# VinAIResearch/COMBAT

Hardware: AMD Instinct MI355X
Metric: images/sec per alternated generator+surrogate step, CIFAR-10 bs=128, 1/2/4/8 GPU (higher is better)
Workload: dtype bf16; 1 GPU; train_generator.py --dataset cifar10 --pc 0.5 --noise_rate 0.08: alternated PreActResNet18 surrogate + UNet generator step (Phase C + Phase G, both Nesterov-SGD updates), bs=128 per GPU, on-device augmentation on; per_gpu_batch=128, global_batch=128, parallelism=dp1 (RCCL all-reduce of netC grads in Phase C, netG grads in Phase G), losses_finite=True, deterministic=True

## Files before the change

combat_amd/_lib.py:

```python
from __future__ import annotations

import ctypes as C
import os

HERE = os.path.dirname(os.path.abspath(__file__))
LIB_PATH = os.environ.get("COMBAT_HIP_LIB") or os.path.join(HERE, "libcombat_hip.so")

c_i32, c_i64, c_f32, c_vp = C.c_int32, C.c_int64, C.c_float, C.c_void_p


class ConvArgs(C.Structure):

    _fields_ = [
        ("N", c_i32), ("H", c_i32), ("W", c_i32), ("C", c_i32),
        ("P", c_i32), ("Q", c_i32), ("K", c_i32),
        ("R", c_i32), ("S", c_i32), ("stride", c_i32), ("pad", c_i32),
        ("mode", c_i32),
        ("src", c_vp), ("wpack", c_vp), ("kpad", c_i32), ("rows_pad", c_i32), ("dst", c_vp),
        ("pro_scale", c_vp), ("pro_shift", c_vp), ("pro_group_stride", c_i32), ("pro_act", c_i32),
        ("pro_slope", c_f32),
        ("bias", c_vp), ("add_pre", c_vp), ("mask_x", c_vp), ("mask_scale", c_vp), ("mask_shift", c_vp),
        ("mask_activated", c_i32), ("mask_group_stride", c_i32), ("mask_slope", c_f32), ("mask_mul_scale", c_i32),
        ("add_post", c_vp), ("tanh_out", c_i32),
        ("stats_kind", c_i32), ("stats", c_vp), ("xh_mean", c_vp), ("xh_rstd", c_vp),
# ... 91 lines not shown
    "combat_head_fwd": (C.c_int, [c_vp, c_i32, c_i32, c_i32, c_vp, c_vp, c_i32, c_vp, c_f32, c_vp, c_vp, c_vp, c_vp,
                                  c_vp, c_vp, c_vp]),
    "combat_head_bwd": (C.c_int, [c_vp, c_i32, c_i32, c_i32, c_vp, c_i32, c_vp, c_vp, c_f32, c_vp, c_vp, c_vp, c_vp,
                                  c_vp]),
    "combat_head_fwd_bwd": (C.c_int, [c_vp, c_i32, c_i32, c_i32, c_vp, c_vp, c_i32, c_vp, c_f32, c_vp, c_vp, c_vp, c_vp,
                                      c_vp, c_vp, c_vp, c_vp, c_vp]),
    "combat_head_bwd_weights": (C.c_int, [c_vp, c_vp, c_i32, c_i32, c_i32, c_i32, c_vp, c_vp, c_vp]),
    "combat_prune_sweep": (C.c_int, [c_vp, c_i32, c_vp, c_vp, c_vp, c_i32, c_i32, c_i32, c_vp, c_vp, c_vp, c_vp, c_vp]),
    "combat_feature_colsum": (C.c_int, [c_vp, c_i32, c_i32, c_vp, c_vp]),
    "combat_strip_superimpose": (C.c_int, [c_vp, c_i32, c_vp, c_i32, c_vp, c_i32, c_i32, c_i32, c_vp, c_vp]),
    "combat_strip_entropy": (C.c_int, [c_vp, c_i32, c_i32, c_i32, c_vp, c_vp]),
    "combat_nc_blend": (C.c_int, [c_vp, c_i32, c_vp, c_i32, c_vp, c_i32, c_i32, c_i32, c_i32, c_vp, c_vp, c_f32, c_vp, c_vp,
                                  c_vp]),
    "combat_nc_update": (C.c_int, [c_vp, c_vp, c_i32, c_vp, c_i32, c_vp, c_i32, c_i32, c_i32, c_i32, c_vp, c_i32, c_i32,
                                   c_vp, c_vp, c_vp, c_vp, c_f32, c_vp, c_f32, c_f32, c_f32, c_f32, c_vp, c_vp, c_vp, c_i32,
                                   c_vp, c_vp]),
    "combat_gradcam_seed": (C.c_int, [c_vp, c_vp, c_i32, c_i32, c_i32, c_i32, c_vp, c_vp, c_vp, c_vp]),
    "combat_gradcam_map": (C.c_int, [c_vp, c_vp, c_i32, c_i32, c_i32, c_i32, c_vp, c_vp, c_vp, c_vp]),
    "combat_comm_unique_id": (C.c_int, [c_vp]),
    "combat_comm_init_rank": (C.c_int, [C.POINTER(c_vp), c_i32, c_vp, c_i32]),
    "combat_comm_destroy": (C.c_int, [c_vp]),
    "combat_allreduce": (C.c_int, [c_vp, c_i64, c_i32, c_vp, c_vp]),
    "combat_sgd_nesterov": (C.c_int, [c_vp, c_vp, c_i32, c_i64, c_f32, c_f32, c_f32, c_f32, c_i32, c_vp]),
    "combat_image_to_c8": (C.c_int, [c_vp, c_i32, c_i32, c_vp, c_vp]),
    "combat_nhwc_to_nchw_f32": (C.c_int, [c_vp, c_i32, c_i32, c_i32, c_i32, c_i32, c_vp, c_vp]),
    "combat_nchw_to_nhwc_bf16": (C.c_int, [c_vp, c_i32, c_i32, c_i32, c_i32, c_i32, c_vp, c_vp]),
    "combat_memset_zero": (C.c_int, [c_vp, c_i64, c_vp]),
    "combat_copy3": (C.c_int, [c_vp, c_vp, c_i64, c_vp, c_vp, c_i64, c_vp, c_vp, c_i64, c_vp]),
    "combat_relu_mask": (C.c_int, [c_vp, c_vp, c_i64, c_vp, c_vp]),
    "combat_colsum": (C.c_int, [c_vp, c_i64, c_i32, c_i32, c_vp, c_vp]),
    "combat_log_terms": (C.c_int, [c_vp, c_vp, c_vp, c_i32, c_i32, c_vp, c_vp, c_vp, c_vp]),
    "combat_log_terms_tv": (C.c_int, [c_vp, c_vp, c_vp, c_vp, c_i32, c_i32, c_vp, c_vp, c_vp, c_vp]),
    "combat_maxpool2": (C.c_int, [c_vp, c_i32, c_i32, c_i32, c_i32, c_vp, c_vp]),
    "combat_elu_affine": (C.c_int, [c_vp, c_i64, c_i32, c_vp, c_vp, c_vp, c_vp]),
    "combat_affine_act": (C.c_int, [c_vp, c_i64, c_i32, c_vp, c_vp, c_i64, c_f32, c_vp, c_vp]),
    "combat_dct_u8": (C.c_int, [c_vp, c_vp, c_i32, c_i32, c_vp, c_vp]),
    "combat_linear_nhwc": (C.c_int, [c_vp, c_i32, c_i32, c_i32, c_i32, c_vp, c_vp, c_i32, c_vp, c_vp]),
    "combat_grid_head_fwd": (C.c_int, [c_vp, c_vp, c_vp, c_i32, c_i32, c_vp, c_vp]),
    "combat_wanet_grid": (C.c_int, [c_vp, c_vp, c_i32, c_i32, c_f32, c_vp, c_vp, c_vp]),
    "combat_warp_fwd": (C.c_int, [c_vp, c_vp, c_vp, c_i32, c_i32, c_i32, c_vp, c_vp]),
    "combat_warp_bwd": (C.c_int, [c_vp, c_vp, c_vp, c_vp, c_i32, c_i32, c_i32, c_i32, c_vp, c_vp]),
    "combat_warp_bwd_input": (C.c_int, [c_vp, c_vp, c_i32, c_i32, c_i32, c_vp, c_vp]),
    "combat_wanet_field_bwd": (C.c_int, [c_vp, c_i32, c_vp, c_vp, c_i32, c_i32, c_f32, c_f32, c_vp, c_vp, c_vp, c_i32, c_vp,
                                         c_vp, c_vp, c_vp, c_vp]),
    "combat_plan_create": (c_vp, []),
    "combat_plan_destroy": (None, [c_vp]),
# ... 45 lines not shown
```

combat_amd/csrc/capi.cpp:

```cpp
#include "combat_hip.h"

#include <hip/hip_runtime.h>

#include <atomic>
#include <cstdlib>
#include <mutex>
#include <unordered_map>

#define COMBAT_ABI_VERSION 21

extern "C" const char *combat_version(void) { return "combat_hip gfx950 abi17"; }
extern "C" int combat_abi_version(void) { return COMBAT_ABI_VERSION; }

static std::atomic<int> g_deterministic{-1};
bool combat_deterministic() {
    int v = g_deterministic.load(std::memory_order_relaxed);
    if (v < 0) {
        const char *e = getenv("COMBAT_DETERMINISTIC");
        v = e && e[0] == '1';
        g_deterministic.store(v, std::memory_order_relaxed);
    }
    return v != 0;
}
extern "C" void combat_set_deterministic(int on) { g_deterministic.store(on ? 1 : 0, std::memory_order_relaxed); }
extern "C" int combat_get_deterministic(void) { return combat_deterministic() ? 1 : 0; }

float *combat_stream_scratch(void *stream, size_t bytes) {
    constexpr size_t kBytes = 2u << 20;
    if (bytes > kBytes) return nullptr;
    static std::mutex mu;
    static std::unordered_map<void *, float *> regions;
    std::lock_guard<std::mutex> lock(mu);
// ... 11 lines not shown
```

combat_amd/csrc/common.hpp:

```cpp
#pragma once
#include <hip/hip_runtime.h>
#include <hip/hip_ext.h>
#include <stdint.h>

#include "combat_hip.h"

typedef __attribute__((ext_vector_type(8))) __bf16 bf16x8_t;
typedef __attribute__((ext_vector_type(4))) float f32x4_t;
typedef __attribute__((ext_vector_type(4))) short s16x4_t;
typedef __attribute__((ext_vector_type(4))) unsigned int u32x4_t;

namespace combat_launch {
extern thread_local hipEvent_t t_stop;
extern thread_local bool t_stop_used;
}
#define COMBAT_LAUNCH(kernel, grid, block, smem, stream, ...)                                             \
    do {                                                                                                  \
        if (hipEvent_t stop_ = combat_launch::t_stop) {                                                   \
            hipExtLaunchKernelGGL(kernel, grid, block, smem, stream, nullptr, stop_, 0, __VA_ARGS__);     \
            combat_launch::t_stop_used = true;                                                            \
        } else {                                                                                          \
            hipLaunchKernelGGL(kernel, grid, block, smem, stream, __VA_ARGS__);                           \
        }                                                                                                 \
    } while (0)
// ... 43 lines not shown
    u[2] = pack_bf16x2(v[4], v[5]);
    u[3] = pack_bf16x2(v[6], v[7]);
    return u;
}

__device__ __forceinline__ uint4 pack8(const float (&v)[8]) {
    uint4 u;
    u.x = pack_bf16x2(v[0], v[1]);
    u.y = pack_bf16x2(v[2], v[3]);
    u.z = pack_bf16x2(v[4], v[5]);
    u.w = pack_bf16x2(v[6], v[7]);
    return u;
}

__device__ __forceinline__ void load8f(const float *p, float (&v)[8]) {
    const float4 a = *reinterpret_cast<const float4 *>(p);
    const float4 b = *reinterpret_cast<const float4 *>(p + 4);
    v[0] = a.x; v[1] = a.y; v[2] = a.z; v[3] = a.w;
    v[4] = b.x; v[5] = b.y; v[6] = b.z; v[7] = b.w;
}

__device__ __forceinline__ float round_bf16(float f) { return bf16_bits_to_f32(f32_to_bf16_bits(f)); }

__device__ __forceinline__ uint4 hilo_pixel(float r, float g, float b) {
    const float hr = round_bf16(r), hg = round_bf16(g), hb = round_bf16(b);
    uint4 u;
    u.x = pack_bf16x2(hr, hg);
    u.y = pack_bf16x2(hb, r - hr);
    u.z = pack_bf16x2(g - hg, b - hb);
    u.w = 0;
    return u;
}

static inline hipStream_t as_stream(void *s) { return reinterpret_cast<hipStream_t>(s); }

bool combat_deterministic();
float *combat_stream_scratch(void *stream, size_t bytes);

static inline int ilog2_exact(int v) {
    if (v <= 0 || (v & (v - 1))) return -1;
    int s = 0;
    while ((1 << s) < v) ++s;
    return s;
}
```

combat_amd/csrc/elementwise.hip:

```cpp
#include "common.hpp"
#include "plan.hpp"

namespace {

__global__ __launch_bounds__(256) void pack_weights_kernel(const float *__restrict__ w, int K, int taps, int creal,
                                                           int C, int dup, __bf16 *__restrict__ wf, int rows_f,
                                                           int kpad_f, __bf16 *__restrict__ wd, int rows_d,
                                                           int kpad_d, int Kc) {
    const long nf = (long)rows_f * kpad_f;
    const long nd = wd ? (long)rows_d * kpad_d : 0;
    for (long t = (long)blockIdx.x * blockDim.x + threadIdx.x; t < nf + nd; t += (long)gridDim.x * blockDim.x) {
        if (t < nf) {
            const int n = (int)(t / kpad_f), k = (int)(t - (long)n * kpad_f);
            const int tap = k / C, c = k - tap * C;
            float v = 0.f;
            if (n < K && tap < taps) {
                int cm = -1;
                if (c < creal) cm = c;
                else if (dup && c < 2 * creal) cm = c - creal;
                if (cm >= 0) v = w[((long)n * taps + tap) * creal + cm];
            }
            wf[t] = (__bf16)v;
        } else {
            const long u = t - nf;
// ... 305 lines not shown
            up_taps(oy, H, y0, y1, wy0, wy1);
            const float wy = (y0 == iy ? wy0 : 0.f) + (y1 == iy ? wy1 : 0.f);
            if (wy == 0.f) continue;
            for (int ox = 2 * ix - 1; ox <= 2 * ix + 2; ++ox) {
                if (ox < 0 || ox >= Wo) continue;
                int x0, x1;
                float wx0, wx1;
                up_taps(ox, W, x0, x1, wx0, wx1);
                const float wx = (x0 == ix ? wx0 : 0.f) + (x1 == ix ? wx1 : 0.f);
                if (wx == 0.f) continue;
                const long off = ((img * Ho + oy) * Wo + ox) * C + c;
                float g[8], o[8];
                unpack8(*reinterpret_cast<const uint4 *>(d_out + off), g);
                unpack8(*reinterpret_cast<const uint4 *>(out + off), o);
                const float wgt = wy * wx;
#pragma unroll
                for (int e = 0; e < 8; ++e) acc[e] = fmaf(wgt * (o[e] > 0.f ? 1.f : 0.2f), g[e], acc[e]);
            }
        }
        *reinterpret_cast<uint4 *>(du + ((img * H + iy) * W + ix) * C + c) = pack8(acc);
    }
}

__global__ __launch_bounds__(256) void sgd_kernel(void *const *__restrict__ ptrs, const int64_t *__restrict__ sizes,
                                                  float lr, float mu, float wd, float gscale, int first) {
    const int t = blockIdx.y;
    float *__restrict__ p = reinterpret_cast<float *>(ptrs[3 * t]);
    const float *__restrict__ g = reinterpret_cast<const float *>(ptrs[3 * t + 1]);
    float *__restrict__ b = reinterpret_cast<float *>(ptrs[3 * t + 2]);
    const long n = sizes[t];
    for (long i = (long)blockIdx.x * blockDim.x + threadIdx.x; i < n; i += (long)gridDim.x * blockDim.x) {
        const float pv = p[i];
        const float gv = fmaf(wd, pv, g[i] * gscale);
        const float bv = first ? gv : fmaf(mu, b[i], gv);
        b[i] = bv;
        p[i] = pv - lr * fmaf(mu, bv, gv);
    }
}

__global__ __launch_bounds__(256) void linear_nhwc_kernel(const __bf16 *__restrict__ x, int h, int w, int C,
                                                          const float *__restrict__ Wt, const float *__restrict__ b,
                                                          int classes, float *__restrict__ logits) {
    __shared__ float red[256];
    const int img = blockIdx.x;
    const int in = C * h * w;
    for (int j = 0; j < classes; ++j) {
        float s = 0.f;
        for (int i = threadIdx.x; i < in; i += 256) {
            const int c = i / (h * w), r = i - c * h * w;
            s = fmaf((float)x[((long)img * h * w + r) * C + c], Wt[(long)j * in + i], s);
        }
        red[threadIdx.x] = s;
        __syncthreads();
        for (int o = 128; o > 0; o >>= 1) {
            if ((int)threadIdx.x < o) red[threadIdx.x] += red[threadIdx.x + o];
            __syncthreads();
        }
        if (threadIdx.x == 0) logits[(long)img * classes + j] = red[0] + b[j];
        __syncthreads();
// ... 364 lines not shown
                                  void *du, void *stream) {
    COMBAT_PLAN_HOOK(combat_unet_up_bwd, d_out, out, N, H, W, C, du);
    if (!d_out || !out || !du || N <= 0 || H <= 0 || W <= 0 || C <= 0 || (C & 7)) return COMBAT_EINVAL;
    COMBAT_LAUNCH(unet_up_bwd_kernel, dim3(grid_for((long)N * H * W * (C / 8), 8192)), dim3(256), 0,
                       as_stream(stream), reinterpret_cast<const __bf16 *>(d_out), reinterpret_cast<const __bf16 *>(out),
                       N, H, W, C, reinterpret_cast<__bf16 *>(du));
    CB_LAUNCH_CHECK();
    return COMBAT_OK;
}

extern "C" int combat_sgd_nesterov(const void *ptrs, const int64_t *sizes, int32_t count, int64_t max_size, float lr,
                                   float momentum, float weight_decay, float grad_scale, int32_t first_step,
                                   void *stream) {
    COMBAT_PLAN_HOOK(combat_sgd_nesterov, ptrs, sizes, count, max_size, lr, momentum, weight_decay, grad_scale, first_step);
    if (!ptrs || !sizes || count <= 0 || max_size <= 0) return COMBAT_EINVAL;
    long bx = (max_size + 255) / 256;
    if (bx > 4096) bx = 4096;
    COMBAT_LAUNCH(sgd_kernel, dim3((unsigned)bx, (unsigned)count), dim3(256), 0, as_stream(stream),
                       reinterpret_cast<void *const *>(ptrs), sizes, lr, momentum, weight_decay, grad_scale, first_step);
    CB_LAUNCH_CHECK();
    return COMBAT_OK;
}

extern "C" int combat_linear_nhwc(const void *x, int32_t n, int32_t h, int32_t w, int32_t C, const float *Wt,
                                  const float *b, int32_t classes, float *logits, void *stream) {
    COMBAT_PLAN_HOOK(combat_linear_nhwc, x, n, h, w, C, Wt, b, classes, logits);
    if (!x || !Wt || !b || !logits || n <= 0 || h <= 0 || w <= 0 || C <= 0 || classes <= 0) return COMBAT_EINVAL;
    COMBAT_LAUNCH(linear_nhwc_kernel, dim3(n), dim3(256), 0, as_stream(stream),
                       reinterpret_cast<const __bf16 *>(x), h, w, C, Wt, b, classes, logits);
    CB_LAUNCH_CHECK();
    return COMBAT_OK;
}
```

combat_amd/csrc/norm.hip:

```cpp
#include "common.hpp"
#include "plan.hpp"

namespace {

constexpr int kStageRows = 64;

__device__ __forceinline__ void reduce_rows(const float *__restrict__ part, int C, int c, long row0, int nrows,
                                            int ry, double &s1, double &s2) {
    s1 = 0.0;
    s2 = 0.0;
    if (c >= C) return;
    for (int r = ry; r < nrows; r += 32) {
        float u[8], v[8];
#pragma unroll
        for (int q = 0; q < 8; ++q) {
            const int rr = r + 4 * q < nrows ? r + 4 * q : r;
            const float *p = part + ((row0 + rr) * 2) * (long)C + c;
            u[q] = p[0];
            v[q] = p[C];
        }
#pragma unroll
        for (int q = 0; q < 8; ++q) {
            if (r + 4 * q < nrows) {
                s1 += (double)u[q];
// ... 88 lines not shown
        const double gm = a.gamma ? (double)a.gamma[c] : 1.0;
        const double mean = a.mean[o], rstd = a.rstd[o];
        const double m1 = s1 / a.count, m2 = s2 / a.count;
        a.ca[o] = (float)(gm * rstd);
        a.cb[o] = (float)(-gm * rstd * rstd * m2);
        a.cc[o] = (float)(gm * rstd * (mean * rstd * m2 - m1));
        if (a.dgamma) a.dgamma[c] = (float)s2;
        if (a.dbeta) a.dbeta[c] = (float)s1;
    }
}

__global__ void bn_eval_fold_kernel(const float *gamma, const float *beta, const float *rm, const float *rv,
                                    float eps, int C, float *scale, float *shift) {
    const int c = blockIdx.x * blockDim.x + threadIdx.x;
    if (c >= C) return;
    const float s = gamma[c] / sqrtf(rv[c] + eps);
    scale[c] = s;
    shift[c] = beta[c] - rm[c] * s;
}

__global__ void bn_eval_fold_batch_kernel(const combat_bn_desc *__restrict__ descs, float eps) {
    const combat_bn_desc d = descs[blockIdx.y];
    for (int c = blockIdx.x * blockDim.x + threadIdx.x; c < d.C; c += gridDim.x * blockDim.x) {
        const float s = d.gamma[c] / sqrtf(d.running_var[c] + eps);
        d.scale[c] = s;
        d.shift[c] = d.beta[c] - d.running_mean[c] * s;
    }
}

__global__ __launch_bounds__(256) void group_stats_kernel(const __bf16 *__restrict__ x, const __bf16 *__restrict__ dz,
                                                          int groups, int rows_per_group, int C, int parts_per_image,
                                                          const float *__restrict__ xh_mean,
                                                          const float *__restrict__ xh_rstd,
                                                          float *__restrict__ part) {
    const int nch = C >> 3;
    const long t = (long)blockIdx.x * blockDim.x + threadIdx.x;
    if (t >= (long)groups * nch) return;
    const int g = (int)(t / nch), c = (int)(t % nch) * 8;
    float s1[8], s2[8], hs[8], hh[8];
#pragma unroll
    for (int e = 0; e < 8; ++e) s1[e] = s2[e] = 0.f;
    if (dz) {
        const long img = parts_per_image > 0 ? g / parts_per_image : 0;
        load8f(xh_rstd + img * C + c, hs);
        load8f(xh_mean + img * C + c, hh);
    }
    for (int r = 0; r < rows_per_group; ++r) {
        const long off = ((long)g * rows_per_group + r) * C + c;
        float xv[8];
// ... 867 lines not shown
```

combat_amd/engine.py:

```python
from __future__ import annotations

import ctypes
import os
from typing import Dict, List, Optional, Tuple

import torch

from . import ops
from ._lib import STATS_PER_WORKGROUP, TILE_D128x32, TILE_D128x64, TILE_S128x64, CombatHipError, ConvArgs, lib
from .nets import UNET_LAYERS
from .ops import Affine, PackedConv, bf16

BATCH_STATS_ROWS = 0 if os.environ.get("COMBAT_STATS_PER_WAVE") == "1" else STATS_PER_WORKGROUP

f32 = torch.float32


def _p(t):
    return None if t is None else t.data_ptr()


class Plan:

    serial = False
# ... 336 lines not shown
        self.sgd_sizes = torch.tensor([self.total], dtype=torch.int64, device=dev)

    def _slice(self, base: torch.Tensor, name: str) -> torch.Tensor:
        o, n, _ = self.offsets[name]
        return base[o:o + n]

    def grad_phys(self, name: str) -> torch.Tensor:
        o, n, shape = self.offsets[name]
        g = self.grad[o:o + n]
        if len(shape) == 4:
            k, c, r, s = shape
            return g.view(k, r * s, c)
        return g.view(shape)

    def logical(self, base: torch.Tensor, name: str) -> torch.Tensor:
        o, n, shape = self.offsets[name]
        g = base[o:o + n]
        if len(shape) == 4:
            k, c, r, s = shape
            return g.view(k, r, s, c).permute(0, 3, 1, 2)
        return g.view(shape)

    zero_ev = None

    def zero_grad_behind(self) -> None:
        if Plan.serial:
            return
        main = torch.cuda.current_stream()
        aux = _aux_stream(main)
        ev = torch.cuda.Event()
        ev.record(main)
        aux.wait_event(ev)
        ops.check(lib.combat_memset_zero(self.grad.data_ptr(), self.total * 4, aux.cuda_stream), "zero_grad")
        self.zero_ev = torch.cuda.Event()
        self.zero_ev.record(aux)

    def sgd_step(self, lr: float, momentum: float = 0.9, weight_decay: float = 5e-4, grad_scale: float = 1.0):
        ops.sgd_nesterov(self.sgd_ptrs, self.sgd_sizes, 1, self.total, lr, momentum, weight_decay, grad_scale, False)




def _zero_grad_call(fp, st):
    ev = fp.zero_ev
    if ev is not None:
        fp.zero_ev = None
        torch.cuda.current_stream().wait_event(ev)
        return 0
    return lib.combat_memset_zero(fp.grad.data_ptr(), fp.total * 4, st)


_SHORT_WORKGROUPS = False


class short_workgroups:

    def __enter__(self):
        global _SHORT_WORKGROUPS
        self.prev, _SHORT_WORKGROUPS = _SHORT_WORKGROUPS, True

    def __exit__(self, *exc):
        global _SHORT_WORKGROUPS
        _SHORT_WORKGROUPS = self.prev


def _tile_preference(a) -> None:
# ... 205 lines not shown
    @flush_at_marks.setter
    def flush_at_marks(self, value: bool) -> None:
        value = bool(value)
        if value != self._flush_at_marks:
            for slot in getattr(self, "slots", {}).values():
                for k in [k for k in slot.plans if k.startswith("bwd")]:
                    del slot.plans[k]
        self._flush_at_marks = value

    def __init__(self, module: torch.nn.Module):
        self.module = module
        self.device = next(module.parameters()).device
        if self.device.type != "cuda":
            raise CombatHipError("combat_amd engines run on the GPU only (module is on %s); there is no CPU path"
                                 % self.device)
        self.fp = FlatParams(module)
        self.convs: List[PackedConv] = []
        self.slots: Dict[Tuple, Slot] = {}
        self._scratch = torch.empty(ops.norm_scratch_bytes(1, 512) // 4, dtype=f32, device=self.device)
        self.weights_dirty = True

    def mark_weights_dirty(self) -> None:
        self.weights_dirty = True

    def slot(self, name: str, n: int, hw: int) -> Slot:
        key = (name, n, hw)
        s = self.slots.get(key)
        if s is None:
            s = Slot(self.device, n, hw)
            self.slots[key] = s
        return s

    def _pc(self, weight, stride, pad, cin_pad, dup=False, need_dgrad=True, row_scale=None) -> PackedConv:
        pc = PackedConv(weight, stride, pad, cin_pad, dup_hilo=dup, need_dgrad=need_dgrad, row_scale=row_scale)
        self.convs.append(pc)
        return pc

    def refresh(self) -> None:
        if not self.weights_dirty:
            return
        self._pack_all()
        self._refresh_extra()
        self.weights_dirty = False

    def _pack_all(self) -> None:
        ptrs = tuple(pc.weight.data_ptr() for pc in self.convs)
        if getattr(self, "_pack_ptrs", None) != ptrs:
            masters = [pc.master() for pc in self.convs]
            if any(m.data_ptr() != q for m, q in zip(masters, ptrs)):
                self._pack_ptrs = None
                for pc in self.convs:
                    pc.pack()
                return
            from ._lib import PackDesc
            tab = (PackDesc * len(self.convs))()
            for d, pc, m in zip(tab, self.convs, masters):
                pc.fill_desc(d, m)
            self._pack_tab = torch.frombuffer(bytearray(bytes(tab)), dtype=torch.uint8).to(self.device)
            self._pack_ptrs = ptrs
        ops.check(lib.combat_pack_weights_batch(self._pack_tab.data_ptr(), len(self.convs),
                                                torch.cuda.current_stream().cuda_stream), "combat_pack_weights_batch")

    def _refresh_extra(self) -> None:
        pass

    FUSED_DIRECT_PX = 1024
    FUSED_MAX_ROWS = 256

    def _norm_scratch(self, plan: Plan, groups: int, c: int, rows: int) -> torch.Tensor:
        if rows > self.FUSED_MAX_ROWS and ops.norm_scratch_bytes(groups, c) > self._scratch.numel() * 4:
            self._scratch = torch.empty(ops.norm_scratch_bytes(groups, c) // 4, dtype=f32, device=self.device)
        plan.hold(self._scratch)
        return self._scratch

    def _conv_norm(self, plan: Plan, slot: Slot, key: str, src, dst, pc: PackedConv, *, groups: int,
                   gamma=None, beta=None, running=None, act_dst=None, slope: float = 0.0, defer: bool = False,
                   **conv_kw) -> NormState:
        n, p, q, c = dst.shape
        pq, m = p * q, n * p * q
        a = ops.conv_args(src, dst, pc, 0, workspace=plan.workspace(src.device), **conv_kw)
        a.stats_kind = 1 | (BATCH_STATS_ROWS if groups == 1 else 0)
        _tile_preference(a)
        rows, rpi = ops.conv_stats_layout(a)
        fused = (groups == 1) or (rpi > 0)
# ... 138 lines not shown

class PreActEngine(NetEngine):

    def __init__(self, module):
        super().__init__(module)
        m = module
        self.classes = m.linear.out_features
        self.stem = self._pc(m.conv1.weight.data, 1, 1, 8, dup=True)
        self.blocks: List[_Blk] = []
        self.bns: List[_BN] = []
        for li in range(1, 5):
            for bi, blk in enumerate(getattr(m, "layer%d" % li)):
                e = _Blk()
                e.prefix = "layer%d.%d." % (li, bi)
                e.stride, e.cin, e.planes = blk.stride, blk.conv1.in_channels, blk.conv1.out_channels
                e.bn1, e.bn2 = _BN(self, blk.bn1, e.prefix + "bn1"), _BN(self, blk.bn2, e.prefix + "bn2")
                e.conv1 = self._pc(blk.conv1.weight.data, blk.stride, 1, e.cin)
                e.conv2 = self._pc(blk.conv2.weight.data, 1, 1, e.planes)
                e.sc = self._pc(blk.shortcut[0].weight.data, blk.stride, 0, e.cin) if hasattr(blk, "shortcut") else None
                self.blocks.append(e)
                self.bns += [e.bn1, e.bn2]
        self.lin_w, self.lin_b = m.linear.weight.data, m.linear.bias.data

    def _refresh_extra(self):
        self.fold_bn()

    def fold_bn(self):
        ptrs = tuple(t.data_ptr() for bn in self.bns for t in (bn.gamma, bn.beta, bn.rm, bn.rv))
        if getattr(self, "_bn_ptrs", None) != ptrs:
            from ._lib import BnDesc
            tab = (BnDesc * len(self.bns))()
            for d, bn in zip(tab, self.bns):
                d.gamma, d.beta, d.running_mean, d.running_var = (t.data_ptr() for t in (bn.gamma, bn.beta, bn.rm, bn.rv))
                d.scale, d.shift, d.C = bn.escale.data_ptr(), bn.eshift.data_ptr(), bn.C
            self._bn_tab = torch.frombuffer(bytearray(bytes(tab)), dtype=torch.uint8).to(self.device)
            self._bn_ptrs = ptrs
        ops.check(lib.combat_bn_eval_fold_batch(self._bn_tab.data_ptr(), len(self.bns), 1e-5,
                                                torch.cuda.current_stream().cuda_stream), "combat_bn_eval_fold_batch")

    def head_bufs(self, slot: Slot):
        n = slot.N
        return dict(
            logits=slot.buf("logits", (n, self.classes), f32), dlogits=slot.buf("dlogits", (n, self.classes), f32),
            pooled=slot.buf("pooled", (n, self.lin_w.shape[1]), f32), loss=slot.buf("loss", (1,), f32, zero=True),
            correct=slot.buf("correct", (2,), torch.int32, zero=True),
            targets=slot.buf("targets", (n,), torch.int64, zero=True),
            targets2=slot.buf("targets2", (n,), torch.int64, zero=True))

    def input(self, slot: Slot) -> torch.Tensor:
        return slot.buf("x", (slot.N, slot.hw, slot.hw, 8))

    FWD_SHARED = ("stem", "logits", "dlogits", "pooled", "targets", "targets2") + tuple(
        "b%d.%s" % (b, s) for b in range(8) for s in ("y1", "out", "sc", "a1", "act")) + ("stem.act",)

    def forward_plan(self, slot: Slot, train: bool, loss_weight: float = 1.0, with_targets2: bool = False,
                     split_head: bool = False, head_bwd: bool = False, two_loss: bool = False, keep_raw_blocks=()) -> Plan:
        keep_raw_blocks = tuple(sorted(set(int(b) for b in keep_raw_blocks)))
        if keep_raw_blocks:
            if type(self) is not PreActEngine or train or two_loss:
# ... 1010 lines not shown
```

combat_amd/ops.py:

```python
from __future__ import annotations

import ctypes
from dataclasses import dataclass
from typing import Optional

import torch

from . import _lib
from ._lib import ConvArgs, WgradArgs, check, lib

bf16 = torch.bfloat16


def _p(t: Optional[torch.Tensor]):
    return None if t is None else t.data_ptr()


def _stream():
    return torch.cuda.current_stream().cuda_stream


def _round_up(v: int, m: int) -> int:
    return (v + m - 1) // m * m

# ... 435 lines not shown
                                  d_feat.data_ptr(), _stream()),
          "combat_gradcam_seed", "n=%d N=%d classes=%d C=%d" % (n, N, classes, c))


def gradcam_map(act, grad, n, cam, raw=None, weights=None) -> None:
    if act.dim() != 4 or act.shape != grad.shape or act.dtype != bf16 or grad.dtype != bf16 or act.shape[1] != act.shape[2] \
            or act.shape[0] < n or not act.is_contiguous() or not grad.is_contiguous():
        raise ValueError("gradcam_map: act and grad must be contiguous bf16 [>= n = %d][f][f][C] of one shape, got %s %s / %s %s"
                         % (n, act.dtype, tuple(act.shape), grad.dtype, tuple(grad.shape)))
    f, c = act.shape[1], act.shape[3]
    for name, v, size in (("cam", cam, n * 32 * 32), ("raw", raw, n * f * f), ("weights", weights, n * c)):
        if v is not None and (v.dtype != torch.float32 or v.numel() < size or not v.is_contiguous()):
            raise ValueError("gradcam_map: %s must be contiguous fp32 with at least %d elements, got %s %s"
                             % (name, size, v.dtype, tuple(v.shape)))
    check(lib.combat_gradcam_map(act.data_ptr(), grad.data_ptr(), n, f, c, 32, cam.data_ptr(), _p(raw), _p(weights), _stream()),
          "combat_gradcam_map", "n=%d f=%d C=%d" % (n, f, c))


def sgd_nesterov(ptrs, sizes, count, max_size, lr, momentum, weight_decay, grad_scale, first_step) -> None:
    check(lib.combat_sgd_nesterov(ptrs.data_ptr(), sizes.data_ptr(), count, max_size, lr, momentum, weight_decay,
                                  grad_scale, int(first_step), _stream()), "combat_sgd_nesterov", "count=%d" % count)


def image_to_c8(x, out_c8) -> None:
    n, _, hw, _ = x.shape
    check(lib.combat_image_to_c8(x.data_ptr(), n, hw, out_c8.data_ptr(), _stream()), "combat_image_to_c8")


def nhwc_to_nchw_f32(x, c, out) -> None:
    n, h, w, cc = x.shape
    check(lib.combat_nhwc_to_nchw_f32(x.data_ptr(), n, h, w, cc, c, out.data_ptr(), _stream()),
          "combat_nhwc_to_nchw_f32")


def nchw_to_nhwc_bf16(x, out) -> None:
    n, c, h, w = x.shape
    check(lib.combat_nchw_to_nhwc_bf16(x.data_ptr(), n, c, h, w, out.shape[-1], out.data_ptr(), _stream()),
          "combat_nchw_to_nhwc_bf16")


def colsum(x, c_out, out) -> None:
    c = x.shape[-1]
    check(lib.combat_colsum(x.data_ptr(), x.numel() // c, c, c_out, out.data_ptr(), _stream()), "combat_colsum")


def maxpool2(x, out) -> None:
# ... 20 lines not shown
```

combat_amd/step.py:

```python
from __future__ import annotations

import contextlib
import copy
import math
from dataclasses import dataclass, field
from types import SimpleNamespace
from typing import Dict, List, Optional

import os

import numpy as np
import torch

from . import ops, trigger
from ._lib import lib
from .augment import PostTensorTransform
from .dist import GradReducer, bucket_ranges
from .engine import (FreqEngine, PlanSeq, PreActEngine, UnetEngine, _zero_grad_call, f32, low_priority_stream,
                     short_workgroups)

BUCKETS = (8, 16, 32, 64, 128, 256, 512, 1024)


def bucket(n: int) -> int:
# ... 348 lines not shown
            self._trigger_c(x_ptr, nb, k1c, st)
        ops.check(lib.combat_augment_fwd(s.cat_src.data_ptr(), s.tab_i[1].data_ptr(), aug_ptr[0], n, hw,
                                         eC.input(s.sC_train).data_ptr(), None, st), "augment 0")
        pl["C_train_f"].run(prof)
        side = self._side_stream()
        side.wait_event(ev_fork)
        xK, xC = eK.input(s.sK_eval), eC.input(s.sC_eval)
        bd_ptr = s.bd.data_ptr()
        with torch.cuda.stream(side):
            s2 = side.cuda_stream
            self._trigger_g(x_ptr, n, k1g, s2)
            ev_bd = torch.cuda.Event()
            ev_bd.record()
            ops.check(lib.combat_augment_fwd(x_ptr, None, aug_ptr[1], n, hw, xK.data_ptr(), None, s2), "augment 1")
            ops.check(lib.combat_augment_fwd(bd_ptr, None, aug_ptr[4], n, hw, xK[n:].data_ptr(), None, s2), "augment 4")
            pl["K_eval_f"].run(prof)
            pl["K_bd_b"].run(prof)
            ops.check(lib.combat_augment_bwd(s.sK_bd.bufs["g.img"].data_ptr(), 8, aug_ptr[4], n, hw,
                                             s.d_bd2.data_ptr(), 0, s2), "augment 4 bwd")
            ev_side = torch.cuda.Event()
            ev_side.record()

        self._backward_allreduce(pl["C_train_b"], eC, prof)
        eC.fp.sgd_step(float(lr_c if lr_c is not None else opt.lr_C), grad_scale=1.0 / self.world)
        if not self.keep_grads:
            eC.fp.zero_grad_behind()
        eC.mark_weights_dirty()
        eC.refresh()

        torch.cuda.current_stream().wait_event(ev_bd)
        self._c_eval_inputs(x_ptr, bd_ptr, xC, aug_ptr, n, st)
        pl["C_eval_f"].run(prof)
        ev_late = torch.cuda.Event()
        ev_late.record()
        pl["C_bd_b"].run(prof)
        self._c_eval_grads(aug_ptr, n, st)
        with torch.cuda.stream(side):
            side.wait_event(ev_late)
            s2 = side.cuda_stream
            if not s.merge_c:
                ops.check(lib.combat_augment_fwd(x_ptr, None, aug_ptr[2], n, hw, eC.input(s.sC_met).data_ptr(), None, s2),
                          "augment 2")
                pl["C_met_f"].run(prof)
            if eF is not None:
                ops.check(lib.combat_dct_u8(bd_ptr, self.D.data_ptr(), n, hw, eF.input(s.sF).data_ptr(), s2), "dct")
                pl["F_f"].run(prof)
            self._log_terms(n, s2, s.sF.bufs["logits"] if eF is not None else None)
            ev_met = torch.cuda.Event()
            ev_met.record()
        torch.cuda.current_stream().wait_event(ev_side)
        self._gen_backward(x_ptr, n, k1g, st, prof)
        eG.fp.sgd_step(float(lr_g if lr_g is not None else opt.lr_G), grad_scale=1.0 / self.world)
        if not self.keep_grads:
            eG.fp.zero_grad_behind()
        eG.mark_weights_dirty()
        torch.cuda.current_stream().wait_event(ev_met)
        self.samples += n
        self.steps_done += 1

    def _draw(self, targets_cpu, bd_targets_cpu) -> StepRandomness:
        return draw_randomness(targets_cpu, bd_targets_cpu, self.opt, self.transforms, self.sigma_range)

    def _gen_forward(self, x_ptr, n, st, prof) -> None:
        s = self.cur
        ops.check(lib.combat_image_to_c8(x_ptr, n, self.hw, self.eG.input(s.sG).data_ptr(), st), "c8 G")
        s.pl["G_f"].run(prof)

    def _trigger_c(self, x_ptr, nb, k1c, st) -> None:
        s = self.cur
        ops.check(lib.combat_trigger_fwd(x_ptr, self.eG.output(s.sG).data_ptr(), self.P.data_ptr(), k1c, float(self.opt.noise_rate),
                                         nb, self.hw, s.tab_i[0].data_ptr(), s.cat_src[s.n:].data_ptr(), None, None, st),
                  "trigger C")

    def _trigger_g(self, x_ptr, n, k1g, s2) -> None:
        s = self.cur
        ops.check(lib.combat_trigger_fwd(x_ptr, self.eG.output(s.sG).data_ptr(), self.P.data_ptr(), k1g, float(self.opt.noise_rate),
                                         n, self.hw, None, s.bd.data_ptr(), None, s.mse.data_ptr(), s2), "trigger G")

# ... 459 lines not shown
            g = self.eG.forward_grid(hw, float(opt.grid_rescale), st)
            ops.check(lib.combat_warp_fwd(s.cat_src.data_ptr(), s.tab_i[0].data_ptr(), g["grid"].data_ptr(), 0, nb, hw,
                                          s.cat_src[n:].data_ptr(), st), "warp")
        elif nb:
            self.eG.refresh()
            nbk = min(bucket(nb), n)
            if nbk not in self._small:
                small = self.eG.slot("V.small", nbk, hw)
                self._small[nbk] = (small, self.eG.forward_plan(small), torch.zeros(nbk, 3, hw, hw, dtype=f32, device=self.dev))
            sS, plan_small, tochange = self._small[nbk]
            self.k1.copy_(torch.from_numpy(trigger.gaussian_kernel1d(
                trigger.sample_sigma(getattr(opt, "sigma", (0.1, 1.0))), opt.kernel_size)))
            ops.check(lib.combat_augment_fwd(s.cat_src.data_ptr(), s.tab_i[0].data_ptr(), None, nbk, hw,
                                             self.eG.input(sS).data_ptr(), tochange.data_ptr(), st), "gather poisoned")
            plan_small.run()
            ops.check(lib.combat_trigger_fwd(tochange.data_ptr(), self.eG.output(sS).data_ptr(), self.P.data_ptr(),
                                             self.k1.data_ptr(), float(opt.noise_rate), nb, hw, None,
                                             s.cat_src[n:].data_ptr(), None, None, st), "trigger")
        ops.check(lib.combat_augment_fwd(s.cat_src.data_ptr(), s.tab_i[1].data_ptr(),
                                         s.tab_f.data_ptr() if aug is not None else None, n, hw,
                                         self.eC.input(s.slot).data_ptr(), None, st), "augment")
        s.fwd.run()
        backward_allreduce(s.bwd, self.eC, self.pg, self.world, self._reducers)
        self.eC.fp.sgd_step(float(lr if lr is not None else opt.lr_C), grad_scale=1.0 / self.world)
        self.eC.mark_weights_dirty()

    def poisoned_pair(self):
        trg, nb = getattr(self, "last_poisoned", (None, 0))
        if not nb:
            return None
        s = self.cur
        return s.cat_src[:s.n][trg.to(self.dev)].clone(), s.cat_src[s.n:s.n + nb].clone()

    def read_metrics(self, reset=False):
        out = {"loss_sum": 0.0, "correct": 0}
        for s in self._sets.values():
            h = self.eC.head_bufs(s.slot)
            out["loss_sum"] += float(h["loss"])
            out["correct"] += int(h["correct"][0])
            if reset:
                h["loss"].zero_()
                h["correct"].zero_()
        return out
```

include/combat_hip.h:

```cpp
#ifndef COMBAT_HIP_H
#define COMBAT_HIP_H

#include <stdint.h>

#ifdef __cplusplus
extern "C" {
#endif

#define COMBAT_OK 0
#define COMBAT_EINVAL (-1)
#define COMBAT_ELAUNCH (-2)

const char *combat_version(void);
int combat_abi_version(void);

void combat_set_deterministic(int on);
int combat_get_deterministic(void);

typedef struct combat_conv_args {
    int32_t N, H, W, C;
    int32_t P, Q, K;
    int32_t R, S, stride, pad;
    int32_t mode;
    const void *src;
// ... 214 lines not shown

int combat_strip_superimpose(const void *backgrounds, int32_t B, const void *dataset, int32_t n_data, const int32_t *index,
                             int32_t S, int32_t hw, int32_t norm_cols, void *out_c8, void *stream);
int combat_strip_entropy(const float *logits, int32_t B, int32_t S, int32_t classes, float *out, void *stream);

int combat_nc_blend(const void *dataset, int32_t n_data, const int32_t *index, int32_t n_index, const int32_t *cursor,
                    int32_t bs, int32_t n, int32_t N, int32_t hw, const float *mask_tanh, const float *pattern_tanh,
                    float epsilon, const float *norm, void *out_c8, void *stream);
int combat_nc_update(const void *g_img, const void *dataset, int32_t n_data, const int32_t *index, int32_t n_index,
                     int32_t *cursor, int32_t bs, int32_t n, int32_t N, int32_t hw, const float *logits, int32_t classes,
                     int32_t target_label, float *mask_tanh, float *pattern_tanh, float *exp_avg, float *exp_avg_sq,
                     float epsilon, const float *norm, float lr, float beta1, float beta2, float adam_eps, int32_t *t,
                     const float *cost, float *stats, int32_t steps, float *grad_out, void *stream);

int combat_gradcam_seed(const float *logits, const int32_t *index, int32_t n, int32_t N, int32_t classes, int32_t C,
                        const float *W, int32_t *chosen, void *d_feat, void *stream);
int combat_gradcam_map(const void *act, const void *grad, int32_t n, int32_t f, int32_t C, int32_t out_hw, float *cam,
                       float *raw, float *weights, void *stream);

int combat_sgd_nesterov(const void *ptrs, const int64_t *sizes, int32_t count, int64_t max_size, float lr,
                        float momentum, float weight_decay, float grad_scale, int32_t first_step,
                        void *stream);

int combat_image_to_c8(const float *x, int32_t n, int32_t hw, void *out_c8, void *stream);
int combat_nhwc_to_nchw_f32(const void *x, int32_t n, int32_t h, int32_t w, int32_t C, int32_t c, float *out,
                            void *stream);
int combat_nchw_to_nhwc_bf16(const float *x, int32_t n, int32_t c, int32_t h, int32_t w, int32_t C, void *out,
                             void *stream);
int combat_relu_mask(const void *g, const void *act, int64_t elements, void *out, void *stream);
int combat_memset_zero(void *ptr, int64_t bytes, void *stream);
int combat_copy3(void *dst0, const void *src0, int64_t bytes0, void *dst1, const void *src1, int64_t bytes1,
                 void *dst2, const void *src2, int64_t bytes2, void *stream);
int combat_colsum(const void *x, int64_t rows, int32_t C, int32_t c_out, float *out, void *stream);
int combat_log_terms(const float *x, const float *xb, const float *mse_partial, int32_t n, int32_t hw,
                     const float *detector_logits, double *acc2, double *hits, void *stream);
int combat_log_terms_tv(const float *x, const float *xb, const float *mse_partial, const float *tv_partial, int32_t n,
                        int32_t hw, const float *detector_logits, double *acc3, double *hits, void *stream);
int combat_maxpool2(const void *x, int32_t n, int32_t h, int32_t w, int32_t C, void *out, void *stream);
int combat_elu_affine(const void *x, int64_t rows, int32_t C, const float *scale, const float *shift, void *out,
                      void *stream);
int combat_affine_act(const void *x, int64_t rows, int32_t C, const float *scale, const float *shift,
                      int64_t group_rows, float slope, void *out, void *stream);
int combat_dct_u8(const float *x, const float *D, int32_t n, int32_t hw, void *out_c8, void *stream);
int combat_linear_nhwc(const void *x, int32_t n, int32_t h, int32_t w, int32_t C, const float *W, const float *b,
                       int32_t classes, float *logits, void *stream);

// ... 39 lines not shown
```

Before: 33150 images/sec.

## Fuse Nesterov SGD update with bf16 weight packing, BN fold and grad zeroing

Adds a single kernel that applies the Nesterov SGD update to the fp32 master weights and, in the same pass, writes the packed bf16 forward and transposed weight layouts, refolds the eval BatchNorm scale and shift, and zeros the gradients. Before, these were separate launches, each reading the full parameter set again. The later zero_grad call is skipped when the grad buffer was already cleared on the same stream. The price is a more complex kernel with a tiled transpose through shared memory and a fallback path for irregular convs, plus extra bookkeeping state (_fused_done, clean_on) that must stay consistent.

New measurement: 33240 images/sec, median of 5. Within noise of the previous version (+0.2%).

```diff
diff --git a/combat_amd/_lib.py b/combat_amd/_lib.py
--- a/combat_amd/_lib.py
+++ b/combat_amd/_lib.py
@@ -137,6 +137,8 @@
     "combat_comm_destroy": (C.c_int, [c_vp]),
     "combat_allreduce": (C.c_int, [c_vp, c_i64, c_i32, c_vp, c_vp]),
     "combat_sgd_nesterov": (C.c_int, [c_vp, c_vp, c_i32, c_i64, c_f32, c_f32, c_f32, c_f32, c_i32, c_vp]),
+    "combat_sgd_nesterov_pack": (C.c_int, [c_vp, c_vp, c_vp, c_i64, c_vp, c_i32, c_vp, c_i32, c_vp, c_i32, c_f32,
+                                           c_f32, c_f32, c_f32, c_f32, c_i32, c_i32, c_vp]),
     "combat_image_to_c8": (C.c_int, [c_vp, c_i32, c_i32, c_vp, c_vp]),
     "combat_nhwc_to_nchw_f32": (C.c_int, [c_vp, c_i32, c_i32, c_i32, c_i32, c_i32, c_vp, c_vp]),
     "combat_nchw_to_nhwc_bf16": (C.c_int, [c_vp, c_i32, c_i32, c_i32, c_i32, c_i32, c_vp, c_vp]),
diff --git a/combat_amd/csrc/capi.cpp b/combat_amd/csrc/capi.cpp
--- a/combat_amd/csrc/capi.cpp
+++ b/combat_amd/csrc/capi.cpp
@@ -7,7 +7,7 @@
 #include <mutex>
 #include <unordered_map>
 
-#define COMBAT_ABI_VERSION 21
+#define COMBAT_ABI_VERSION 22
 
 extern "C" const char *combat_version(void) { return "combat_hip gfx950 abi17"; }
 extern "C" int combat_abi_version(void) { return COMBAT_ABI_VERSION; }
diff --git a/combat_amd/csrc/common.hpp b/combat_amd/csrc/common.hpp
--- a/combat_amd/csrc/common.hpp
+++ b/combat_amd/csrc/common.hpp
@@ -89,6 +89,13 @@
 
 __device__ __forceinline__ float round_bf16(float f) { return bf16_bits_to_f32(f32_to_bf16_bits(f)); }
 
+__device__ __forceinline__ void bn_eval_fold_one(float gamma, float beta, float mean, float var, float eps, float &scale,
+                                                 float &shift) {
+    const float s = gamma / sqrtf(var + eps);
+    scale = s;
+    shift = beta - mean * s;
+}
+
 __device__ __forceinline__ uint4 hilo_pixel(float r, float g, float b) {
     const float hr = round_bf16(r), hg = round_bf16(g), hb = round_bf16(b);
     uint4 u;
diff --git a/combat_amd/csrc/elementwise.hip b/combat_amd/csrc/elementwise.hip
--- a/combat_amd/csrc/elementwise.hip
+++ b/combat_amd/csrc/elementwise.hip
@@ -351,6 +351,17 @@
     }
 }
 
+struct SgdScalars {
+    float lr, mu, wd, gscale;
+    int first;
+};
+
+__device__ __forceinline__ void sgd_update(const SgdScalars &s, float &p, float g, float &b) {
+    const float gv = fmaf(s.wd, p, g * s.gscale);
+    b = s.first ? gv : fmaf(s.mu, b, gv);
+    p = p - s.lr * fmaf(s.mu, b, gv);
+}
+
 __global__ __launch_bounds__(256) void sgd_kernel(void *const *__restrict__ ptrs, const int64_t *__restrict__ sizes,
                                                   float lr, float mu, float wd, float gscale, int first) {
     const int t = blockIdx.y;
@@ -358,12 +369,150 @@
     const float *__restrict__ g = reinterpret_cast<const float *>(ptrs[3 * t + 1]);
     float *__restrict__ b = reinterpret_cast<float *>(ptrs[3 * t + 2]);
     const long n = sizes[t];
+    const SgdScalars s{lr, mu, wd, gscale, first};
     for (long i = (long)blockIdx.x * blockDim.x + threadIdx.x; i < n; i += (long)gridDim.x * blockDim.x) {
-        const float pv = p[i];
-        const float gv = fmaf(wd, pv, g[i] * gscale);
-        const float bv = first ? gv : fmaf(mu, b[i], gv);
+        float pv = p[i], bv = b[i];
+        sgd_update(s, pv, g[i], bv);
         b[i] = bv;
-        p[i] = pv - lr * fmaf(mu, bv, gv);
+        p[i] = pv;
+    }
+}
+
+struct SgdPackArgs {
+    float *p, *g, *b;
+    const combat_pack_desc *descs;
+    const int64_t *segs;
+    const combat_bn_desc *bns;
+    int n_desc, n_seg, n_bn;
+    float eps;
+    int zero;
+    SgdScalars s;
+};
+
+__device__ __forceinline__ void sgd_one(const SgdPackArgs &a, long i) {
+    float pv = a.p[i], bv = a.b[i];
+    sgd_update(a.s, pv, a.g[i], bv);
+    a.b[i] = bv;
+    a.p[i] = pv;
+    if (a.zero) a.g[i] = 0.f;
+}
+
+__device__ __forceinline__ void store8f(float *p, const float (&v)[8]) {
+    *reinterpret_cast<float4 *>(p) = make_float4(v[0], v[1], v[2], v[3]);
+    *reinterpret_cast<float4 *>(p + 4) = make_float4(v[4], v[5], v[6], v[7]);
+}
+
+__global__ __launch_bounds__(256) void sgd_pack_kernel(const SgdPackArgs a) {
+    __shared__ float tile[64][65];
+    const int tid = threadIdx.x;
+    int row = blockIdx.y;
+    if (row >= a.n_desc + a.n_seg) {
+        const combat_bn_desc d = a.bns[row - a.n_desc - a.n_seg];
+        const long og = d.gamma - a.p, ob = d.beta - a.p;
+        for (int c = blockIdx.x * blockDim.x + tid; c < d.C; c += gridDim.x * blockDim.x) {
+            sgd_one(a, og + c);
+            sgd_one(a, ob + c);
+            bn_eval_fold_one(a.p[og + c], a.p[ob + c], d.running_mean[c], d.running_var[c], a.eps, d.scale[c], d.shift[c]);
+        }
+        return;
+    }
+    if (row >= a.n_desc) {
+        row -= a.n_desc;
+        const long o = a.segs[2 * row], n = a.segs[2 * row + 1];
+        for (long i = (long)blockIdx.x * blockDim.x + tid; i < n; i += (long)gridDim.x * blockDim.x) sgd_one(a, o + i);
+        return;
+    }
+    const combat_pack_desc d = a.descs[row];
+    const long off = d.w - a.p;
+    __bf16 *__restrict__ wf = reinterpret_cast<__bf16 *>(d.wf);
+    __bf16 *__restrict__ wd = reinterpret_cast<__bf16 *>(d.wd);
+    const int K = d.K, taps = d.taps, creal = d.c_real, C = d.C, Kc = (d.K + 7) & ~7;
+    if (creal == C && !d.dup_hilo && d.kpad_f == taps * C && !d.row_scale && !(K & 7)) {
+        float *p = a.p + off, *g = a.g + off, *b = a.b + off;
+        const long nreal = (long)K * d.kpad_f, nf = (long)d.rows_pad_f * d.kpad_f;
+        for (long t8 = nreal + ((long)blockIdx.x * blockDim.x + tid) * 8; t8 < nf; t8 += (long)gridDim.x * blockDim.x * 8)
+            *reinterpret_cast<uint4 *>(wf + t8) = make_uint4(0u, 0u, 0u, 0u);
+        const int tiles_k = wd ? d.kpad_d / 64 : (taps * Kc + 63) / 64;
+        const int tiles_c = ((wd ? d.rows_pad_d : C) + 63) / 64;
+        const int kl = tid >> 3, c8 = (tid & 7) * 8;
+        const int cl = tid >> 2, k16 = (tid & 3) * 16;
+        for (int tl = blockIdx.x; tl < tiles_k * tiles_c; tl += gridDim.x) {
+            const int c0 = (tl / tiles_k) * 64, k0 = (tl % tiles_k) * 64, c = c0 + c8;
+            float v[2][8], gv[2][8], bv[2][8];
+            long m[2];
+            bool in[2];
+#pragma unroll
+            for (int h = 0; h < 2; ++h) {
+                const int k = k0 + kl + 32 * h, tap = k / Kc, n = k - tap * Kc;
+                in[h] = tap < taps && n < K && c < C;
+                m[h] = ((long)n * taps + tap) * C + c;
+                if (in[h]) {
+                    load8f(p + m[h], v[h]);
+                    load8f(g + m[h], gv[h]);
+                    load8f(b + m[h], bv[h]);
+                }
+            }
+#pragma unroll
+            for (int h = 0; h < 2; ++h) {
+                if (in[h]) {
+#pragma unroll
+                    for (int e = 0; e < 8; ++e) sgd_update(a.s, v[h][e], gv[h][e], bv[h][e]);
+                    store8f(p + m[h], v[h]);
+                    store8f(b + m[h], bv[h]);
+                    if (a.zero) {
+                        *reinterpret_cast<float4 *>(g + m[h]) = make_float4(0.f, 0.f, 0.f, 0.f);
+                        *reinterpret_cast<float4 *>(g + m[h] + 4) = make_float4(0.f, 0.f, 0.f, 0.f);
+                    }
+                    *reinterpret_cast<uint4 *>(wf + m[h]) = pack8(v[h]);
+                } else {
+#pragma unroll
+                    for (int e = 0; e < 8; ++e) v[h][e] = 0.f;
+                }
+            }
+            if (wd) {
+#pragma unroll
+                for (int h = 0; h < 2; ++h)
+#pragma unroll
+                    for (int e = 0; e < 8; ++e) tile[kl + 32 * h][c8 + e] = v[h][e];
+                __syncthreads();
+                if (c0 + cl < d.rows_pad_d) {
+                    __bf16 *dst = wd + (long)(c0 + cl) * d.kpad_d + k0 + k16;
+#pragma unroll
+                    for (int h = 0; h < 2; ++h) {
+                        float o[8];
+#pragma unroll
+                        for (int e = 0; e < 8; ++e) o[e] = tile[k16 + 8 * h + e][cl];
+                        *reinterpret_cast<uint4 *>(dst + 8 * h) = pack8(o);
+                    }
+                }
+                __syncthreads();
+            }
+        }
+        return;
+    }
+    if (blockIdx.x) return;
+    const long nel = (long)K * taps * creal;
+    for (long i = tid; i < nel; i += blockDim.x) sgd_one(a, off + i);
+    __syncthreads();
+    const float *w = a.p + off;
+    const float *rs = d.row_scale;
+    const long nf = (long)d.rows_pad_f * d.kpad_f, nd = wd ? (long)d.rows_pad_d * d.kpad_d : 0;
+    for (long t = tid; t < nf; t += blockDim.x) {
+        const int n = (int)(t / d.kpad_f), k = (int)(t - (long)n * d.kpad_f);
+        const int tap = k / C, c = k - tap * C;
+        float v = 0.f;
+        if (n < K && tap < taps) {
+            int cm = -1;
+            if (c < creal) cm = c;
+            else if (d.dup_hilo && c < 2 * creal) cm = c - creal;
+            if (cm >= 0) v = w[((long)n * taps + tap) * creal + cm] * (rs ? rs[n] : 1.f);
+        }
+        wf[t] = (__bf16)v;
+    }
+    for (long u = tid; u < nd; u += blockDim.x) {
+        const int c = (int)(u / d.kpad_d), k = (int)(u - (long)c * d.kpad_d);
+        const int tap = k / Kc, n = k - tap * Kc;
+        wd[u] = (__bf16)((c < creal && tap < taps && n < K) ? w[((long)n * taps + tap) * creal + c] * (rs ? rs[n] : 1.f) : 0.f);
     }
 }
 
@@ -774,6 +923,29 @@
     return COMBAT_OK;
 }
 
+extern "C" int combat_sgd_nesterov_pack(float *master, float *grad, float *momentum_buf, int64_t total,
+                                        const combat_pack_desc *descs, int32_t n_desc, const int64_t *segments,
+                                        int32_t n_segments, const combat_bn_desc *bns, int32_t n_bn, float bn_eps,
+                                        float lr, float momentum, float weight_decay, float grad_scale,
+                                        int32_t first_step, int32_t zero_grad, void *stream) {
+    COMBAT_PLAN_HOOK(combat_sgd_nesterov_pack, master, grad, momentum_buf, total, descs, n_desc, segments, n_segments, bns,
+                     n_bn, bn_eps, lr, momentum, weight_decay, grad_scale, first_step, zero_grad);
+    if (!master || !grad || !momentum_buf || total <= 0 || n_desc < 0 || n_segments < 0 || n_bn < 0) return COMBAT_EINVAL;
+    if ((n_desc && !descs) || (n_segments && !segments) || (n_bn && !bns)) return COMBAT_EINVAL;
+    const long rows = (long)n_desc + n_segments + n_bn;
+    if (rows <= 0 || rows > 65535) return COMBAT_EINVAL;
+    SgdPackArgs a;
+    a.p = master, a.g = grad, a.b = momentum_buf;
+    a.descs = descs, a.segs = segments, a.bns = bns;
+    a.n_desc = n_desc, a.n_seg = n_segments, a.n_bn = n_bn;
+    a.eps = bn_eps;
+    a.zero = zero_grad != 0;
+    a.s = SgdScalars{lr, momentum, weight_decay, grad_scale, first_step};
+    COMBAT_LAUNCH(sgd_pack_kernel, dim3(288, (unsigned)rows), dim3(256), 0, as_stream(stream), a);
+    CB_LAUNCH_CHECK();
+    return COMBAT_OK;
+}
+
 extern "C" int combat_linear_nhwc(const void *x, int32_t n, int32_t h, int32_t w, int32_t C, const float *Wt,
                                   const float *b, int32_t classes, float *logits, void *stream) {
     COMBAT_PLAN_HOOK(combat_linear_nhwc, x, n, h, w, C, Wt, b, classes, logits);
diff --git a/combat_amd/csrc/norm.hip b/combat_amd/csrc/norm.hip
--- a/combat_amd/csrc/norm.hip
+++ b/combat_amd/csrc/norm.hip
@@ -134,9 +134,7 @@
 __global__ void bn_eval_fold_batch_kernel(const combat_bn_desc *__restrict__ descs, float eps) {
     const combat_bn_desc d = descs[blockIdx.y];
     for (int c = blockIdx.x * blockDim.x + threadIdx.x; c < d.C; c += gridDim.x * blockDim.x) {
-        const float s = d.gamma[c] / sqrtf(d.running_var[c] + eps);
-        d.scale[c] = s;
-        d.shift[c] = d.beta[c] - d.running_mean[c] * s;
+        bn_eval_fold_one(d.gamma[c], d.beta[c], d.running_mean[c], d.running_var[c], eps, d.scale[c], d.shift[c]);
     }
 }
 
diff --git a/combat_amd/engine.py b/combat_amd/engine.py
--- a/combat_amd/engine.py
+++ b/combat_amd/engine.py
@@ -382,6 +382,10 @@
         return g.view(shape)
 
     zero_ev = None
+    clean_on = None
+
+    def mark_grad_dirty(self) -> None:
+        self.clean_on = None
 
     def zero_grad_behind(self) -> None:
         if Plan.serial:
@@ -402,6 +406,9 @@
 
 
 def _zero_grad_call(fp, st):
+    clean, fp.clean_on = fp.clean_on, None
+    if clean is not None and clean == st and fp.zero_ev is None:
+        return 0
     ev = fp.zero_ev
     if ev is not None:
         fp.zero_ev = None
@@ -653,6 +660,7 @@
 
     def mark_weights_dirty(self) -> None:
         self.weights_dirty = True
+        self._fused_done = 0
 
     def slot(self, name: str, n: int, hw: int) -> Slot:
         key = (name, n, hw)
@@ -670,27 +678,91 @@
     def refresh(self) -> None:
         if not self.weights_dirty:
             return
-        self._pack_all()
-        self._refresh_extra()
+        done, self._fused_done = self._fused_done, 0
+        if done < 1:
+            self._pack_all()
+        if done < 2:
+            self._refresh_extra()
         self.weights_dirty = False
 
-    def _pack_all(self) -> None:
+    def _pack_table(self) -> bool:
         ptrs = tuple(pc.weight.data_ptr() for pc in self.convs)
         if getattr(self, "_pack_ptrs", None) != ptrs:
             masters = [pc.master() for pc in self.convs]
             if any(m.data_ptr() != q for m, q in zip(masters, ptrs)):
                 self._pack_ptrs = None
-                for pc in self.convs:
-                    pc.pack()
-                return
+                return False
             from ._lib import PackDesc
             tab = (PackDesc * len(self.convs))()
             for d, pc, m in zip(tab, self.convs, masters):
                 pc.fill_desc(d, m)
             self._pack_tab = torch.frombuffer(bytearray(bytes(tab)), dtype=torch.uint8).to(self.device)
             self._pack_ptrs = ptrs
+        return True
+
+    def _pack_all(self) -> None:
+        if not self._pack_table():
+            for pc in self.convs:
+                pc.pack()
+            return
         ops.check(lib.combat_pack_weights_batch(self._pack_tab.data_ptr(), len(self.convs),
                                                 torch.cuda.current_stream().cuda_stream), "combat_pack_weights_batch")
+
+    fused_update = True
+    fused_zero_grad = True
+    _fused_done = 0
+    _extra_is_fold = False
+
+    def _fused_tables(self):
+        if not self.convs or not self._pack_table():
+            return None
+        bns = self.bns if self._extra_is_fold else []
+        if bns:
+            self._bn_table()
+        key = (self._pack_ptrs, getattr(self, "_bn_ptrs", None) if bns else None)
+        if getattr(self, "_fused_key", None) != key:
+            self._fused_key, self._fused_tab = key, None
+            fp = self.fp
+            base, owned = fp.flat.data_ptr(), []
+            ok = not any(pc.row_scale is not None for pc in self.convs)
+            for pc in self.convs:
+                owned.append(((pc.weight.data_ptr() - base) // 4, pc.K * pc.taps * pc.c_real))
+            for bn in bns:
+                owned += [((t.data_ptr() - base) // 4, bn.C) for t in (bn.gamma, bn.beta)]
+            ok = ok and all((p - base) % 32 == 0 for p in self._pack_ptrs)
+            if ok:
+                try:
+                    segs = ops.plain_segments(fp.total, owned)
+                except ValueError:
+                    segs = None
+                if segs is not None:
+                    seg_t = torch.tensor(segs, dtype=torch.int64, device=self.device).view(-1, 2) if segs else None
+                    self._fused_tab = (seg_t, len(bns))
+        return self._fused_tab
+
+    def sgd_step_and_refresh(self, lr: float, momentum: float = 0.9, weight_decay: float = 5e-4, grad_scale: float = 1.0,
+                             zero_grad: bool = True, refresh: bool = True) -> None:
+        fp = self.fp
+        tabs = self._fused_tables() if self.fused_update else None
+        if tabs is None:
+            fp.sgd_step(lr, momentum, weight_decay, grad_scale)
+            if zero_grad:
+                fp.zero_grad_behind()
+            self.mark_weights_dirty()
+        else:
+            segs, n_bn = tabs
+            zero = zero_grad and self.fused_zero_grad
+            ops.sgd_nesterov_pack(fp.flat, fp.grad, fp.mom, self._pack_tab, len(self.convs), segs,
+                                  self._bn_tab if n_bn else None, n_bn, 1e-5, lr, momentum, weight_decay, grad_scale,
+                                  False, zero)
+            if zero:
+                fp.clean_on = torch.cuda.current_stream().cuda_stream
+            elif zero_grad:
+                fp.zero_grad_behind()
+            self.weights_dirty = True
+            self._fused_done = 2 if (n_bn and self._extra_is_fold) or type(self)._refresh_extra is NetEngine._refresh_extra else 1
+        if refresh:
+            self.refresh()
 
     def _refresh_extra(self) -> None:
         pass
@@ -875,10 +947,12 @@
                 self.bns += [e.bn1, e.bn2]
         self.lin_w, self.lin_b = m.linear.weight.data, m.linear.bias.data
 
+    _extra_is_fold = True
+
     def _refresh_extra(self):
         self.fold_bn()
 
-    def fold_bn(self):
+    def _bn_table(self) -> None:
         ptrs = tuple(t.data_ptr() for bn in self.bns for t in (bn.gamma, bn.beta, bn.rm, bn.rv))
         if getattr(self, "_bn_ptrs", None) != ptrs:
             from ._lib import BnDesc
@@ -888,6 +962,9 @@
                 d.scale, d.shift, d.C = bn.escale.data_ptr(), bn.eshift.data_ptr(), bn.C
             self._bn_tab = torch.frombuffer(bytearray(bytes(tab)), dtype=torch.uint8).to(self.device)
             self._bn_ptrs = ptrs
+
+    def fold_bn(self):
+        self._bn_table()
         ops.check(lib.combat_bn_eval_fold_batch(self._bn_tab.data_ptr(), len(self.bns), 1e-5,
                                                 torch.cuda.current_stream().cuda_stream), "combat_bn_eval_fold_batch")
 
diff --git a/combat_amd/ops.py b/combat_amd/ops.py
--- a/combat_amd/ops.py
+++ b/combat_amd/ops.py
@@ -481,6 +481,33 @@
                                   grad_scale, int(first_step), _stream()), "combat_sgd_nesterov", "count=%d" % count)
 
 
+def plain_segments(total: int, owned) -> list:
+    segs, at = [], 0
+    for o, n in sorted(owned):
+        if n <= 0 or o < at or o + n > total:
+            raise ValueError("range (%d, %d) overlaps its predecessor or leaves [0, %d)" % (o, n, total))
+        if o > at:
+            segs.append((at, o - at))
+        at = o + n
+    if at < total:
+        segs.append((at, total - at))
+    return segs
+
+
+def sgd_nesterov_pack(flat, grad, mom, pack_tab, n_desc, segments, bn_tab, n_bn, bn_eps, lr, momentum, weight_decay,
+                      grad_scale, first_step, zero_grad) -> None:
+    if not (flat.numel() == grad.numel() == mom.numel()) or any(t.dtype != torch.float32 or not t.is_contiguous()
+                                                                 for t in (flat, grad, mom)):
+        raise ValueError("sgd_nesterov_pack: flat, grad and mom must be contiguous fp32 tensors of one length")
+    n_seg = 0 if segments is None else segments.shape[0]
+    if n_seg and (segments.dtype != torch.int64 or not segments.is_contiguous() or segments.shape[1] != 2):
+        raise ValueError("sgd_nesterov_pack: segments must be a contiguous int64 [n, 2] tensor")
+    check(lib.combat_sgd_nesterov_pack(flat.data_ptr(), grad.data_ptr(), mom.data_ptr(), flat.numel(), _p(pack_tab), n_desc,
+                                       _p(segments) if n_seg else None, n_seg, _p(bn_tab) if n_bn else None, n_bn, bn_eps,
+                                       lr, momentum, weight_decay, grad_scale, int(first_step), int(zero_grad), _stream()),
+          "combat_sgd_nesterov_pack", "total=%d convs=%d segments=%d bns=%d" % (flat.numel(), n_desc, n_seg, n_bn))
+
+
 def image_to_c8(x, out_c8) -> None:
     n, _, hw, _ = x.shape
     check(lib.combat_image_to_c8(x.data_ptr(), n, hw, out_c8.data_ptr(), _stream()), "combat_image_to_c8")
diff --git a/combat_amd/step.py b/combat_amd/step.py
--- a/combat_amd/step.py
+++ b/combat_amd/step.py
@@ -394,11 +394,8 @@
             ev_side.record()
 
         self._backward_allreduce(pl["C_train_b"], eC, prof)
-        eC.fp.sgd_step(float(lr_c if lr_c is not None else opt.lr_C), grad_scale=1.0 / self.world)
-        if not self.keep_grads:
-            eC.fp.zero_grad_behind()
-        eC.mark_weights_dirty()
-        eC.refresh()
+        eC.sgd_step_and_refresh(float(lr_c if lr_c is not None else opt.lr_C), grad_scale=1.0 / self.world,
+                                zero_grad=not self.keep_grads)
 
         torch.cuda.current_stream().wait_event(ev_bd)
         self._c_eval_inputs(x_ptr, bd_ptr, xC, aug_ptr, n, st)
@@ -422,10 +419,8 @@
             ev_met.record()
         torch.cuda.current_stream().wait_event(ev_side)
         self._gen_backward(x_ptr, n, k1g, st, prof)
-        eG.fp.sgd_step(float(lr_g if lr_g is not None else opt.lr_G), grad_scale=1.0 / self.world)
-        if not self.keep_grads:
-            eG.fp.zero_grad_behind()
-        eG.mark_weights_dirty()
+        eG.sgd_step_and_refresh(float(lr_g if lr_g is not None else opt.lr_G), grad_scale=1.0 / self.world,
+                                zero_grad=not self.keep_grads, refresh=False)
         torch.cuda.current_stream().wait_event(ev_met)
         self.samples += n
         self.steps_done += 1
@@ -931,8 +926,8 @@
                                          self.eC.input(s.slot).data_ptr(), None, st), "augment")
         s.fwd.run()
         backward_allreduce(s.bwd, self.eC, self.pg, self.world, self._reducers)
-        self.eC.fp.sgd_step(float(lr if lr is not None else opt.lr_C), grad_scale=1.0 / self.world)
-        self.eC.mark_weights_dirty()
+        self.eC.sgd_step_and_refresh(float(lr if lr is not None else opt.lr_C), grad_scale=1.0 / self.world,
+                                     zero_grad=False, refresh=False)
 
     def poisoned_pair(self):
         trg, nb = getattr(self, "last_poisoned", (None, 0))
diff --git a/include/combat_hip.h b/include/combat_hip.h
--- a/include/combat_hip.h
+++ b/include/combat_hip.h
@@ -260,6 +260,12 @@
                         float momentum, float weight_decay, float grad_scale, int32_t first_step,
                         void *stream);
 
+int combat_sgd_nesterov_pack(float *master, float *grad, float *momentum_buf, int64_t total,
+                             const combat_pack_desc *descs, int32_t n_desc, const int64_t *segments, int32_t n_segments,
+                             const combat_bn_desc *bns, int32_t n_bn, float bn_eps,
+                             float lr, float momentum, float weight_decay, float grad_scale, int32_t first_step,
+                             int32_t zero_grad, void *stream);
+
 int combat_image_to_c8(const float *x, int32_t n, int32_t hw, void *out_c8, void *stream);
 int combat_nhwc_to_nchw_f32(const void *x, int32_t n, int32_t h, int32_t w, int32_t C, int32_t c, float *out,
                             void *stream);
```
